# sdwyc/ROLO

Hardware: AMD Instinct MI355X
Metric: scans/sec (128k-pt frame, 20 GN iters) (higher is better)
Workload: dtype f64

## Files before the change

rolo_amd/csrc/knn_packet.hpp:

```cpp
#pragma once
#include "rolo_internal.hpp"
#include "dev_math.hpp"
#include <cfloat>
#include <climits>

#ifndef KNN_STAT
#ifdef ROLO_KNN_STATS
#define KNN_STAT(x) x
#else
#define KNN_STAT(x)
#endif
#endif

namespace rolo {
namespace {

constexpr int WALK_STACK = KNN_WALK_STACK;

ROLO_DEV float box_d2(const float4& lo, const float4& hi, const float4& q) {
  float dx = fmaxf(fmaxf(__fsub_rn(lo.x, q.x), __fsub_rn(q.x, hi.x)), 0.f);
  float dy = fmaxf(fmaxf(__fsub_rn(lo.y, q.y), __fsub_rn(q.y, hi.y)), 0.f);
  float dz = fmaxf(fmaxf(__fsub_rn(lo.z, q.z), __fsub_rn(q.z, hi.z)), 0.f);
  return __fadd_rn(__fadd_rn(__fmul_rn(dx, dx), __fmul_rn(dy, dy)), __fmul_rn(dz, dz));
}

ROLO_DEV double key_pack(float d2, int idx) {
  return __longlong_as_double((long long)(((unsigned long long)__float_as_uint(d2) << 32) | (unsigned)idx));
}
ROLO_DEV float key_d2(double k) { return __uint_as_float((unsigned)((unsigned long long)__double_as_longlong(k) >> 32)); }
ROLO_DEV int key_idx(double k) { return (int)(unsigned)((unsigned long long)__double_as_longlong(k) & 0xffffffffull); }

ROLO_DEV double vmin_f64(double a, double b) { double r; asm("v_min_f64 %0, %1, %2" : "=v"(r) : "v"(a), "v"(b)); return r; }
ROLO_DEV double vmax_f64(double a, double b) { double r; asm("v_max_f64 %0, %1, %2" : "=v"(r) : "v"(a), "v"(b)); return r; }
#ifndef ROLO_KNN_SPLIT_MINMAX
ROLO_DEV void insert_slot(double& ks, double ksm1, double c) { asm("v_min_f64 %0, %1, %0\n\tv_max_f64 %0, %2, %0" : "+&v"(ks) : "v"(c), "v"(ksm1)); }
#else
ROLO_DEV void insert_slot(double& ks, double ksm1, double c) { ks = vmax_f64(ksm1, vmin_f64(c, ks)); }
#endif
#ifndef ROLO_KNN_B1
#define ROLO_KNN_B1 15
#define ROLO_KNN_B2 10
#define ROLO_KNN_B3 5
#endif
template <int KMAX>
ROLO_DEV void insert_tiered(double (&K)[KMAX], double ck) {
  constexpr int B1 = KMAX == 20 ? ROLO_KNN_B1 : 3 * (KMAX / 4), B2 = KMAX == 20 ? ROLO_KNN_B2 : 2 * (KMAX / 4), B3 = KMAX == 20 ? ROLO_KNN_B3 : KMAX / 4;
#pragma unroll
  for (int s = KMAX - 1; s >= B1; s--) insert_slot(K[s], K[s - 1], ck);
  if (__any(ck < K[B1 - 1])) {
#pragma unroll
    for (int s = B1 - 1; s >= B2; s--) insert_slot(K[s], K[s - 1], ck);
    if (__any(ck < K[B2 - 1])) {
#pragma unroll
      for (int s = B2 - 1; s >= B3; s--) insert_slot(K[s], K[s - 1], ck);
      if (__any(ck < K[B3 - 1])) {
#pragma unroll
        for (int s = B3 - 1; s >= 1; s--) insert_slot(K[s], K[s - 1], ck);
        K[0] = vmin_f64(ck, K[0]);
      }
    }
  }
}

ROLO_DEV void sload_leaf(const float4* __restrict__ p, float4 (&pts)[KNN_LEAF]) {
#pragma unroll
  for (int u = 0; u < KNN_LEAF; u++) pts[u] = p[u];
}
ROLO_DEV void sload_node(const float4* __restrict__ p, float4& llo, float4& lhi, float4& rlo, float4& rhi) { llo = p[0]; lhi = p[1]; rlo = p[2]; rhi = p[3]; }

template <int KMAX, bool LOWER = false>
ROLO_DEV void knn_score_leaf(const float4* __restrict__ sorted, int g, const float4& q, double (&K)[KMAX], int kk, double& bkey, float& bd,
                             unsigned& n_ins, unsigned& lane_acc, unsigned& rounds, double lo = 0.0) {
  float4 pts[KNN_LEAF];
  sload_leaf(sorted + KNN_LEAF * (size_t)g, pts);
  KNN_STAT(const double bkey0 = bkey; unsigned my_acc = 0;)
#ifdef ROLO_KNN_STATS2
  unsigned my_cur = 0;
#endif
#pragma unroll
  for (int u = 0; u < KNN_LEAF; u++) {
    const float4 c = pts[u];
    const float dx = q.x - c.x, dy = q.y - c.y, dz = q.z - c.z;
    const float cd = ((dx * dx) + (dy * dy)) + (dz * dz);
    const double ck0 = key_pack(cd, __float_as_int(c.w));
    const double ck = (LOWER && !(ck0 > lo)) ? key_pack(INFINITY, INT_MAX) : ck0;
    KNN_STAT(if (__any(ck < bkey)) { n_ins++; lane_acc += (unsigned)__popcll(__ballot(ck < bkey)); })
    KNN_STAT(if (ck < bkey0) my_acc++;)
#ifdef ROLO_KNN_STATS2
    if (ck < bkey) my_cur++;
#endif
    if (ck < bkey) {
      insert_tiered<KMAX>(K, ck);
#pragma unroll
      for (int s = 0; s < KMAX; s++) if (s == kk - 1) bkey = K[s];
      bd = key_d2(bkey);
    }
  }
#ifdef ROLO_KNN_STATS
#ifdef ROLO_KNN_STATS2
  rounds += my_cur;
  (void)my_acc;
#else
  { unsigned m = my_acc;
    for (int off = 32; off > 0; off >>= 1) m = max(m, (unsigned)__shfl_xor((int)m, off, 64));
    rounds += m; }
#endif
#endif
}

template <int CTRL>
ROLO_DEV double dpp_f64(double x) {
  const long long v = __double_as_longlong(x);
  const int lo = __builtin_amdgcn_mov_dpp((int)(unsigned)(unsigned long long)v, CTRL, 0xF, 0xF, true);
  const int hi = __builtin_amdgcn_mov_dpp((int)(unsigned)((unsigned long long)v >> 32), CTRL, 0xF, 0xF, true);
  return __longlong_as_double((long long)(((unsigned long long)(unsigned)hi << 32) | (unsigned)lo));
}
template <int ST> ROLO_DEV double sub_xchg(double x) { return ST == 0 ? dpp_f64<0xB1>(x) : ST == 1 ? dpp_f64<0x4E>(x) : dpp_f64<0x141>(x); }
template <int SUB> ROLO_DEV double sub_min(double x) {
  x = vmin_f64(x, sub_xchg<0>(x));
  if (SUB >= 4) x = vmin_f64(x, sub_xchg<1>(x));
  if (SUB >= 8) x = vmin_f64(x, sub_xchg<2>(x));
  return x;
}
template <int SUB> ROLO_DEV double sub_max(double x) {
  x = vmax_f64(x, sub_xchg<0>(x));
  if (SUB >= 4) x = vmax_f64(x, sub_xchg<1>(x));
  if (SUB >= 8) x = vmax_f64(x, sub_xchg<2>(x));
  return x;
}

ROLO_DEV int xcd_contiguous_block(int b, int G, int wpb = 4) {
#ifdef ROLO_KNN_NO_XCD_REMAP
  return b;
#else
  if (G * wpb <= 2048) {
    const int x = b & 7, k = b >> 3, q = G >> 3, r = G & 7;
    return x * q + min(x, r) + k;
  }
  const int RUN = 256 / wpb, GROUP = 8 * RUN;
  if (b >= G / GROUP * GROUP) return b;
  const int grp = b / GROUP, o = b - grp * GROUP;
  return grp * GROUP + (o & 7) * RUN + (o >> 3);
#endif
}

typedef __attribute__((address_space(3))) int lds_int;

template <int KMAX, bool LOWER>
ROLO_DEV void packet_walk(const float4* __restrict__ sorted, const float4* __restrict__ boxes, int P, int g_own0, int g_own1, const float4& q, double (&K)[KMAX], int kk,
                          double& bkey, float& bd, double lo, lds_int* stk, int& sp, int h,
                          unsigned& st_nodes, unsigned& st_leaves, unsigned& st_ins, unsigned& st_lane, unsigned& st_rounds, unsigned& st_push) {
  (void)st_push;
  while (true) {
    h = __builtin_amdgcn_readfirstlane(h);
    if (h < P) {
      st_nodes++;
      float4 llo, lhi, rlo, rhi;
      sload_node(boxes + 4 * (size_t)h, llo, lhi, rlo, rhi);
      const float bl = box_d2(llo, lhi, q), br = box_d2(rlo, rhi, q);
      const bool okl = (bl <= bd) && (bl < INFINITY), okr = (br <= bd) && (br < INFINITY);
      const unsigned long long ml = __ballot(okl), mr = __ballot(okr);
      if (ml != 0ull && mr != 0ull) {
        const unsigned long long pref = __ballot((okl || okr) && (bl <= br));
        const bool left_first = 2 * __popcll(pref) >= __popcll(ml | mr);
        if (sp < WALK_STACK) { stk[sp] = left_first ? 2 * h + 1 : 2 * h; sp++; KNN_STAT(st_push++;) }
        h = left_first ? 2 * h : 2 * h + 1;
        continue;
      }
      if (ml != 0ull) { h = 2 * h; continue; }
      if (mr != 0ull) { h = 2 * h + 1; continue; }
    } else {
      const int g = h - P;
      if (g < g_own0 || g >= g_own1) {
        knn_score_leaf<KMAX, LOWER>(sorted, g, q, K, kk, bkey, bd, st_ins, st_lane, st_rounds, lo);
        st_leaves++;
      }
    }
    if (sp == 0) return;
    sp--;
    h = stk[sp];
  }
}

}
}
```

rolo_amd/csrc/knn_walk.hpp:

```cpp
#pragma once
#ifdef ROLO_KNN_STATS
#define KNN_STAT(x) x
#else
#define KNN_STAT(x)
#endif
#include "knn_packet.hpp"

namespace rolo {
namespace {

ROLO_DEV double* stage_area(const KnnCloud& cl, unsigned add) {
  double* s = cl.stage;
  if (cl.stage_epoch) {
    const unsigned long long e = __hip_atomic_load(cl.stage_epoch, __ATOMIC_RELAXED, __HIP_MEMORY_SCOPE_SYSTEM) + add;
    if (e & 1ull) s += cl.stage_alt;
  }
  return s;
}

#ifdef ROLO_KNN_STATS
__device__ unsigned g_knn_wave_rec[16384][8];
#endif

template <int KMAX>
ROLO_DEV void walk_write_lists(const KnnCloud& cl, const double (&K)[KMAX], int kk, double bkey, int qi, int j) {
  int ki[KMAX];
#pragma unroll
  for (int u = 0; u < KMAX; u++) ki[u] = key_idx(K[u]);
  const int slot0 = (KMAX == 64) ? cl.slot0 : 0;
  const int ktot = (KMAX == 64 && cl.k_total) ? cl.k_total : kk;
  if (cl.knn_idx) {
#pragma unroll
    for (int u = 0; u < KMAX; u++) if (u < kk) { cl.knn_idx[(size_t)qi * ktot + slot0 + u] = ki[u]; cl.knn_d2[(size_t)qi * ktot + slot0 + u] = key_d2(K[u]); }
  }
  if (KMAX == 64 && cl.lower) cl.lower[j] = bkey;
  int32_t* __restrict__ nbr = cl.nbr;
#pragma unroll
  for (int u = 0; u < KMAX; u++) nbr[(size_t)(slot0 + u) * cl.n_sorted + j] = ki[u];
}

template <int KMAX>
ROLO_DEV void walk_write_moments(const KnnCloud& cl, const double (&K)[KMAX], int kk, int qi, int j, int (*s_ki)[256]) {
  if (cl.knn_idx) {
#pragma unroll
    for (int u = 0; u < KMAX; u++) if (u < kk) { cl.knn_idx[(size_t)qi * kk + u] = key_idx(K[u]); cl.knn_d2[(size_t)qi * kk + u] = key_d2(K[u]); }
  }
  const int tid = threadIdx.x;
#pragma unroll
  for (int u = 0; u < KMAX; u++) s_ki[u][tid] = key_idx(K[u]);
  const float4* __restrict__ orig = cl.xyz;
  double mx = 0, my = 0, mz = 0;
#pragma unroll 5
  for (int u = 0; u < kk; u++) { const float4 p = orig[s_ki[u][tid]]; mx += (double)p.x; my += (double)p.y; mz += (double)p.z; }
  mx /= kk; my /= kk; mz /= kk;
  double cxx = 0, cxy = 0, cxz = 0, cyy = 0, cyz = 0, czz = 0;
#pragma unroll 5
  for (int u = 0; u < kk; u++) {
    const float4 p = orig[s_ki[u][tid]];
    const double ax = (double)p.x - mx, ay = (double)p.y - my, az = (double)p.z - mz;
    cxx += ax * ax; cxy += ax * ay; cxz += ax * az; cyy += ay * ay; cyz += ay * az; czz += az * az;
  }
  double* __restrict__ mom = reinterpret_cast<double*>(cl.nbr);
  const size_t pitch = (size_t)cl.n_sorted;
  mom[j] = cxx / kk; mom[pitch + j] = cxy / kk; mom[2 * pitch + j] = cxz / kk; mom[3 * pitch + j] = cyy / kk; mom[4 * pitch + j] = cyz / kk; mom[5 * pitch + j] = czz / kk;
}

#ifndef ROLO_KNN_WALK_OCC
#define ROLO_KNN_WALK_OCC 4
#endif
#ifndef ROLO_KNN_PACKET
#define ROLO_KNN_PACKET 64
#endif
#ifndef ROLO_KNN_SEED_EXTRA
#define ROLO_KNN_SEED_EXTRA 1
#endif
static_assert(ROLO_KNN_PACKET == 64, "one query per lane");

template <int KMAX, bool LOWER>
ROLO_DEV void walk_seeds(const float4* __restrict__ sorted, int g_mine0, int g_own0, int g_own1, int n_leaves, const float4& q, double (&K)[KMAX], int kk, double& bkey, float& bd, double lo,
                         unsigned& st_leaves, unsigned& st_ins, unsigned& st_lane, unsigned& st_rounds) {
  const int n_own = min(g_mine0 + 64 / KNN_LEAF, n_leaves) - g_mine0, n_before = g_mine0 - g_own0;
  for (int i = 0; i < g_own1 - g_own0; i++) {
    const int g = i < n_own ? g_mine0 + i : (i - n_own < n_before ? g_own0 + (i - n_own) : g_mine0 + (i - n_before));
    knn_score_leaf<KMAX, LOWER>(sorted, g, q, K, kk, bkey, bd, st_ins, st_lane, st_rounds, lo);
    st_leaves++;
  }
}

template <int KMAX, bool LOWER = false, bool MOMENTS = false>
__global__ __launch_bounds__(256, KMAX > 32 ? 2 : (MOMENTS ? 6 : ROLO_KNN_WALK_OCC)) void knn_walk_kernel(KnnPair A, int split, int k) {
  __shared__ int stk[4][WALK_STACK];
  __shared__ int s_ki[MOMENTS ? KMAX : 1][256];
  const int tid = threadIdx.x;
  const int wv = tid >> 6;
  const int blk = xcd_contiguous_block((int)blockIdx.x, (int)gridDim.x, 4);
  const int which = blk >= split ? 1 : 0;
  const float4* __restrict__ sorted = A.c[which].sorted;
  const float4* __restrict__ boxes = A.c[which].boxes;
  const int n_sorted = A.c[which].n_sorted, P = A.c[which].P;
  const int lane_ = tid & 63;
  const int j = A.c[which].q_begin + (blk - (which ? split : 0)) * 256 + wv * 64 + lane_;
  float4 q = make_float4(0.f, 0.f, 0.f, 0.f);
  int qi = INT_MAX;
  if (j < A.c[which].q_end) { q = sorted[j]; qi = __float_as_int(q.w); }
  const bool active = qi != INT_MAX;
  const int kk = (KMAX == 20) ? 20 : k;
  const int n_leaves = n_sorted / KNN_LEAF;
  unsigned st_nodes = 0, st_leaves = 0, st_ins = 0, st_lane = 0, st_rounds = 0, st_push = 0;

  const double sentinel = key_pack(INFINITY, INT_MAX);
  double K[KMAX];
#pragma unroll
  for (int u = 0; u < KMAX; u++) K[u] = sentinel;
  float bd = active ? INFINITY : -1.0f;
  double bkey = active ? sentinel : key_pack(0.f, 0);

  const int g_mine0 = __builtin_amdgcn_readfirstlane(j / KNN_LEAF);
  const int g_own0 = max(g_mine0 - ROLO_KNN_SEED_EXTRA, 0);
  const int g_own1 = min(g_mine0 + 64 / KNN_LEAF + ROLO_KNN_SEED_EXTRA, n_leaves);
  double lo = 0.0;
  if (LOWER && active) lo = A.c[which].lower[j];
  (void)lo;
  walk_seeds<KMAX, LOWER>(sorted, g_mine0, g_own0, g_own1, n_leaves, q, K, kk, bkey, bd, lo, st_leaves, st_ins, st_lane, st_rounds);

  int sp = 0;
  int h = 1;
#ifdef ROLO_KNN_STATS
  unsigned long long wt0;
  asm("s_memrealtime %0\n\ts_waitcnt lgkmcnt(0)\n\ts_mov_b32 %1, 1" : "=s"(wt0), "=s"(h));
#endif
  packet_walk<KMAX, LOWER>(sorted, boxes, P, g_own0, g_own1, q, K, kk, bkey, bd, lo, (lds_int*)&stk[wv][0], sp, h, st_nodes, st_leaves, st_ins, st_lane, st_rounds, st_push);
#ifdef ROLO_KNN_STATS
  { unsigned long long wt1; asm volatile("s_memrealtime %0\n\ts_waitcnt lgkmcnt(0)" : "=s"(wt1));
    unsigned st_rounds_rec = st_rounds;
#ifdef ROLO_KNN_STATS2
    for (int off = 32; off > 0; off >>= 1) st_rounds_rec = max(st_rounds_rec, (unsigned)__shfl_xor((int)st_rounds_rec, off, 64));
#endif
    const unsigned wid = blockIdx.x * 4 + (threadIdx.x >> 6);
    if ((threadIdx.x & 63) == 0 && wid < 16384) {
      g_knn_wave_rec[wid][0] = st_nodes; g_knn_wave_rec[wid][1] = st_leaves; g_knn_wave_rec[wid][2] = st_ins; g_knn_wave_rec[wid][3] = st_push;
      g_knn_wave_rec[wid][4] = (unsigned)wt0; g_knn_wave_rec[wid][5] = (unsigned)wt1; g_knn_wave_rec[wid][6] = st_lane; g_knn_wave_rec[wid][7] = st_rounds_rec;
    } }
#endif
  (void)st_nodes; (void)st_leaves; (void)st_ins; (void)st_lane; (void)st_rounds; (void)st_push;

  if (!active) return;

  if (MOMENTS) {
    walk_write_moments<KMAX>(A.c[which], K, kk, qi, j, s_ki);
    return;
  }
  walk_write_lists<KMAX>(A.c[which], K, kk, bkey, qi, j);
}

template <int ST> ROLO_DEV void merge20(double (&K)[20]) {
#pragma unroll
  for (int j = 0; j < 10; j++) {
    const double o1 = sub_xchg<ST>(K[19 - j]), o2 = sub_xchg<ST>(K[j]);
    K[j] = vmin_f64(K[j], o1);
    K[19 - j] = vmin_f64(K[19 - j], o2);
  }
#pragma unroll
  for (int d = 16; d >= 1; d >>= 1) {
#pragma unroll
    for (int p = 12; p < 32; p++) {
      if ((p & d) == 0) {
        const int x = p - 12, y = p + d - 12;
        const double lo = vmin_f64(K[x], K[y]);
        K[y] = vmax_f64(K[x], K[y]);
        K[x] = lo;
      }
    }
  }
}

template <int SUB, bool MOMENTS = false>
__global__ __launch_bounds__(256, MOMENTS ? 6 : ROLO_KNN_WALK_OCC) void knn_walk_sub_kernel(KnnPair A, int split ) {
  constexpr int SH = SUB == 2 ? 1 : 2, QPW = 64 / SUB, PPL = KNN_LEAF / SUB, KMAX = 20, E = 4 / SUB , OWN = QPW / KNN_LEAF;
  static_assert(SUB == 2 || SUB == 4, "lanes per query");
  static_assert(KNN_LEAF == 16, "a wavefront's queries are whole leaves");
  __shared__ int stk_[4][WALK_STACK];
  __shared__ int s_ki[MOMENTS ? KMAX : 1][256];
  const int tid = threadIdx.x;
  const int wv = __builtin_amdgcn_readfirstlane(tid >> 6), lane = tid & 63, sub = lane & (SUB - 1), ql = lane >> SH;
  const int blk = xcd_contiguous_block((int)blockIdx.x, (int)gridDim.x, 4);
  const int which = blk >= split ? 1 : 0;
  const KnnCloud& cl = A.c[which];
  const float4* __restrict__ sorted = cl.sorted;
  const float4* __restrict__ boxes = cl.boxes;
  const int n_sorted = cl.n_sorted, P = cl.P, n_leaves = n_sorted / KNN_LEAF;
  const int j0 = cl.q_begin + ((blk - (which ? split : 0)) * 4 + wv) * QPW;
  const int j = j0 + ql;
  float4 q = make_float4(0.f, 0.f, 0.f, 0.f);
  int qi = INT_MAX;
  if (j < cl.q_end) { q = sorted[j]; qi = __float_as_int(q.w); }
  const bool active = qi != INT_MAX;
  const double sentinel = key_pack(INFINITY, INT_MAX);
  double K[KMAX];
#pragma unroll
  for (int u = 0; u < KMAX; u++) K[u] = sentinel;
  double B = active ? sentinel : key_pack(0.f, 0);
  float bd = active ? INFINITY : -1.0f;
  auto score = [&](int g) {
    const float4* __restrict__ leaf = sorted + KNN_LEAF * (size_t)g;
    bool changed = false;
#pragma unroll
    for (int t0 = 0; t0 < PPL; t0 += 4) {
      float4 c[4];
#pragma unroll
      for (int t = 0; t < 4; t++) c[t] = leaf[(t0 + t) * SUB + sub];
#pragma unroll
      for (int t = 0; t < 4; t++) {
        const float dx = q.x - c[t].x, dy = q.y - c[t].y, dz = q.z - c[t].z;
        const float cd = ((dx * dx) + (dy * dy)) + (dz * dz);
        const double ck = key_pack(cd, __float_as_int(c[t].w));
        if (ck < B) { insert_tiered<KMAX>(K, ck); changed = true; }
      }
    }
    if (__any(changed)) {
      B = vmin_f64(vmin_f64(B, sub_min<SUB>(K[KMAX - 1])), sub_max<SUB>(K[KMAX / SUB - 1]));
      bd = key_d2(B);
    }
  };
  const int g_mine = min(j0 / KNN_LEAF, n_leaves - 1);
  const int g_own0 = max(g_mine - ROLO_KNN_SEED_EXTRA, 0), g_own1 = min(g_mine + OWN + ROLO_KNN_SEED_EXTRA, n_leaves);
  for (int g = g_mine; g < min(g_mine + OWN, n_leaves); g++) score(g);
  for (int g = g_own0; g < g_own1; g++) if (g < g_mine || g >= g_mine + OWN) score(g);
  {
    lds_int* stk = (lds_int*)&stk_[wv][0];
    int sp = 0, h = 1;
    while (true) {
      h = __builtin_amdgcn_readfirstlane(h);
      if (2 * h < P) {
        float d[E]; bool ok[E];
        float dm = INFINITY;
#pragma unroll
        for (int e = 0; e < E; e++) {
          const int c = sub * E + e;
          const float4 blo = boxes[8 * (size_t)h + 2 * c], bhi = boxes[8 * (size_t)h + 2 * c + 1];
          d[e] = box_d2(blo, bhi, q);
          ok[e] = (d[e] <= bd) && (d[e] < INFINITY);
          dm = fminf(dm, ok[e] ? d[e] : INFINITY);
        }
        dm = fminf(dm, __int_as_float(__builtin_amdgcn_mov_dpp(__float_as_int(dm), 0xB1, 0xF, 0xF, true)));
        if (SUB == 4) dm = fminf(dm, __int_as_float(__builtin_amdgcn_mov_dpp(__float_as_int(dm), 0x4E, 0xF, 0xF, true)));
        unsigned long long m[E], v[E];
#pragma unroll
        for (int e = 0; e < E; e++) { m[e] = __ballot(ok[e]); v[e] = __ballot(ok[e] && d[e] == dm); }
        int key[4];
#pragma unroll
        for (int c = 0; c < 4; c++) {
          const unsigned long long sel = (SUB == 4 ? 0x1111111111111111ull : 0x5555555555555555ull) << (c / E);
          key[c] = (m[c % E] & sel) != 0ull ? __popcll(v[c % E] & sel) * 4 + (3 - c) : -1;
        }
        auto cx = [](int& a, int& bb) { const int hi = max(a, bb), lo = min(a, bb); a = hi; bb = lo; };
        cx(key[0], key[1]); cx(key[2], key[3]); cx(key[0], key[2]); cx(key[1], key[3]); cx(key[1], key[2]);
        if (key[0] >= 0) {
#pragma unroll
          for (int r = 3; r >= 1; r--) if (key[r] >= 0 && sp < WALK_STACK) { stk[sp] = 4 * h + (3 - (key[r] & 3)); sp++; }
          h = 4 * h + (3 - (key[0] & 3));
          continue;
        }
      } else if (h < P) {
        const int c = sub & 1;
        const float4 blo = boxes[4 * (size_t)h + 2 * c], bhi = boxes[4 * (size_t)h + 2 * c + 1];
        const float d = box_d2(blo, bhi, q);
        const float o = __int_as_float(__builtin_amdgcn_mov_dpp(__float_as_int(d), 0xB1, 0xF, 0xF, true));
        const bool ok = (d <= bd) && (d < INFINITY), oko = (o <= bd) && (o < INFINITY);
        const unsigned long long m = __ballot(ok);
        const unsigned long long ml = m & 0x5555555555555555ull, mr = m & 0xaaaaaaaaaaaaaaaaull;
        if (ml != 0ull && mr != 0ull) {
          const unsigned long long pref = __ballot(c == 0 && (ok || oko) && (d <= o));
          const unsigned long long either = (ml | (mr >> 1)) & 0x5555555555555555ull;
          const bool left_first = 2 * __popcll(pref) >= __popcll(either);
          if (sp < WALK_STACK) { stk[sp] = left_first ? 2 * h + 1 : 2 * h; sp++; }
          h = left_first ? 2 * h : 2 * h + 1;
          continue;
        }
        if (ml != 0ull) { h = 2 * h; continue; }
        if (mr != 0ull) { h = 2 * h + 1; continue; }
      } else {
        const int g = h - P;
        if (g < g_own0 || g >= g_own1) score(g);
      }
      if (sp == 0) break;
      sp--;
      h = stk[sp];
    }
  }
  merge20<0>(K);
  if (SUB == 4) merge20<1>(K);
  if (MOMENTS) {
    if (active && sub == 0) walk_write_moments<KMAX>(cl, K, KMAX, qi, j, s_ki);
    return;
  }
  constexpr int NS = KMAX / SUB;
  int ki[NS];
#pragma unroll
  for (int t = 0; t < NS; t++) {
    if (SUB == 4) {
      const double k01 = sub & 1 ? K[NS + t] : K[t], k23 = sub & 1 ? K[3 * NS + t] : K[2 * NS + t];
      ki[t] = key_idx(sub & 2 ? k23 : k01);
    } else {
      ki[t] = key_idx(sub & 1 ? K[NS + t] : K[t]);
    }
  }
  if (!active) return;
  int32_t* __restrict__ nbr = cl.nbr;
#pragma unroll
  for (int t = 0; t < NS; t++) nbr[(size_t)(sub * NS + t) * n_sorted + j] = ki[t];
  if (cl.knn_idx && sub == 0) {
#pragma unroll
    for (int u = 0; u < KMAX; u++) { cl.knn_idx[(size_t)qi * KMAX + u] = key_idx(K[u]); cl.knn_d2[(size_t)qi * KMAX + u] = key_d2(K[u]); }
  }
}

#ifndef ROLO_KNN_TAIL_OCC
#define ROLO_KNN_TAIL_OCC 2
#endif
template <int KMAX, bool MOMENTS = false>
__global__ __launch_bounds__(256, ROLO_KNN_TAIL_OCC) void knn_tail_kernel(KnnPair A, int split, int k, int reg, VoxelFuse vf) {
  ROLO_TAIL_KERNEL_PRIO();
  int which, blk;
  {
    const int b = xcd_contiguous_block((int)blockIdx.x, (int)gridDim.x), nb0 = split, nb1 = (int)gridDim.x - split, m = nb0 < nb1 ? nb0 : nb1;
    if (b < 2 * m) { which = b & 1; blk = (b >> 1) + (which ? split : 0); }
    else { which = nb0 > nb1 ? 0 : 1; blk = m + (b - 2 * m) + (which ? split : 0); }
  }
  const KnnCloud& cl = A.c[which];
  const int n_sorted = cl.n_sorted;
  const int j = cl.q_begin + (blk - (which ? split : 0)) * 256 + threadIdx.x;
  const bool fuse = vf.enabled && which == vf.which && !cl.stage;
  float4 sp = make_float4(0.f, 0.f, 0.f, 0.f);
  int qi = INT_MAX;
  if (j < cl.q_end) { sp = cl.sorted[j]; qi = __float_as_int(sp.w); }
  const bool act = qi != INT_MAX;
  if (!act && !fuse) return;
  int vox_id = -1;
  if (fuse && act) { const int slot = vf.tgt_slot[qi]; if (slot >= 0) vox_id = slot_id(vf.tab, (unsigned)slot); }
  double c6[6] = {0, 0, 0, 0, 0, 0};
  if (act && MOMENTS) {
    const size_t pitch = (size_t)n_sorted;
    const double* __restrict__ cv = reinterpret_cast<const double*>(cl.nbr);
    const double m0 = cv[j], m1 = cv[pitch + j], m2 = cv[2 * pitch + j], m3 = cv[3 * pitch + j], m4 = cv[4 * pitch + j], m5 = cv[5 * pitch + j];
    if (cl.stage) {
      double* o = stage_area(cl, 1) + (size_t)(j / cl.chunk) * cl.seg + cl.stage_off + (size_t)(j % cl.chunk) * 6;
      knn_covariance_finish(m0, m1, m2, m3, m4, m5, 1, 0, reg, o, c6);
    } else {
      knn_covariance_finish(m0, m1, m2, m3, m4, m5, cl.n, qi, reg, cl.cov, c6, cl.nrm);
    }
  } else if (act) {
    const int32_t* __restrict__ nbr = cl.nbr;
    int ki[KMAX];
#pragma unroll
    for (int u = 0; u < KMAX; u++) ki[u] = nbr[(size_t)u * n_sorted + j];
    if (cl.stage) {
      double* o = stage_area(cl, 1) + (size_t)(j / cl.chunk) * cl.seg + cl.stage_off + (size_t)(j % cl.chunk) * 6;
      knn_covariance_tail<KMAX>(ki, (KMAX == 20) ? 20 : k, cl.xyz, 1, 0, reg, o, c6);
    } else {
      knn_covariance_tail<KMAX>(ki, (KMAX == 20) ? 20 : k, cl.xyz, cl.n, qi, reg, cl.cov, c6, cl.nrm);
    }
  }
#ifdef ROLO_VOXEL_ACCUM_WAVE
  if (fuse) accumulate_point(vf.tab, vox_id, sp, c6, fix_scales(cl.n, vf.counters), true, const_cast<int*>(vf.counters) + 1);
#else
  if (fuse) accumulate_point_wg<256>(vf.tab, vox_id, sp, c6, fix_scales(cl.n, vf.counters), const_cast<int*>(vf.counters) + 1);
#endif
}

__global__ __launch_bounds__(256) void knn_tail_loop_kernel(KnnPair A, int split, int k, int reg, VoxelFuse vf) {
  const int blk = xcd_contiguous_block((int)blockIdx.x, (int)gridDim.x);
  const int which = blk >= split ? 1 : 0;
  const KnnCloud& cl = A.c[which];
  const int j = cl.q_begin + (blk - (which ? split : 0)) * 256 + threadIdx.x;
  const bool fuse = vf.enabled && which == vf.which && !cl.stage;
  float4 sp = make_float4(0.f, 0.f, 0.f, 0.f);
  int qi = INT_MAX;
  if (j < cl.q_end) { sp = cl.sorted[j]; qi = __float_as_int(sp.w); }
  const bool act = qi != INT_MAX;
  if (!act && !fuse) return;
  double c6[6] = {0, 0, 0, 0, 0, 0};
  if (act) {
    if (cl.stage) {
      double* o = stage_area(cl, 1) + (size_t)(j / cl.chunk) * cl.seg + cl.stage_off + (size_t)(j % cl.chunk) * 6;
      knn_covariance_tail_loop(cl.nbr, (size_t)cl.n_sorted, j, k, cl.xyz, 1, 0, reg, o, c6);
    } else {
      knn_covariance_tail_loop(cl.nbr, (size_t)cl.n_sorted, j, k, cl.xyz, cl.n, qi, reg, cl.cov, c6, cl.nrm);
    }
  }
  if (fuse) {
    int id = -1;
    if (act) { const int slot = vf.tgt_slot[qi]; if (slot >= 0) id = slot_id(vf.tab, (unsigned)slot); }
    accumulate_point_wg<256>(vf.tab, id, sp, c6, fix_scales(cl.n, vf.counters), const_cast<int*>(vf.counters) + 1);
  }
}

__global__ __launch_bounds__(256) void knn_unstage_kernel(KnnPair A, int split, int own_only, VoxelFuse vf) {
  const int which = (int)blockIdx.x >= split ? 1 : 0;
  const KnnCloud& cl = A.c[which];
  const int j = (own_only ? cl.q_begin : 0) + ((int)blockIdx.x - (which ? split : 0)) * 256 + threadIdx.x;
  const bool fuse = vf.enabled && which == vf.which;
  float4 sp = make_float4(0.f, 0.f, 0.f, 0.f);
  int qi = INT_MAX;
  if (j < (own_only ? cl.q_end : cl.n_sorted)) { sp = cl.sorted[j]; qi = __float_as_int(sp.w); }
  const bool act = qi != INT_MAX;
  if (!act && !fuse) return;
  double c6[6] = {0, 0, 0, 0, 0, 0};
  if (act) {
    const double* __restrict__ o = stage_area(cl, 0) + (size_t)(j / cl.chunk) * cl.seg + cl.stage_off + (size_t)(j % cl.chunk) * 6;
    const size_t pitch = (size_t)cl.n;
#pragma unroll
    for (int v = 0; v < 6; v++) { c6[v] = o[v]; cl.cov[v * pitch + qi] = c6[v]; }
  }
  if (fuse) {
    int id = -1;
    if (act) { const int slot = vf.tgt_slot[qi]; if (slot >= 0) id = slot_id(vf.tab, (unsigned)slot); }
    accumulate_point_wg<256>(vf.tab, id, sp, c6, fix_scales(cl.n, vf.counters), const_cast<int*>(vf.counters) + 1);
  }
}

}
}
```

Baseline: 4237.

## Seed KNN lists with branch-free sorting-network merges instead of per-point inserts

Seed-leaf scoring now sorts each chunk of 8 (or 4) candidate keys with a fixed sorting network and merges it into the top-20 list with bitonic clean passes, replacing per-point tiered insertion with its data-dependent branches and ballots. The bound is refreshed once after all seed leaves instead of after every insert. The aim is to cut wavefront divergence and per-point branch overhead during seeding. In exchange it always does the full compare-exchange work even when a candidate would be rejected, and it skips the early bound tightening that could prune later points.

```diff
diff --git a/rolo_amd/csrc/knn_packet.hpp b/rolo_amd/csrc/knn_packet.hpp
--- a/rolo_amd/csrc/knn_packet.hpp
+++ b/rolo_amd/csrc/knn_packet.hpp
@@ -1,6 +1,7 @@
 #pragma once
 #include "rolo_internal.hpp"
 #include "dev_math.hpp"
+#include "knn_seed_net.hpp"
 #include <cfloat>
 #include <climits>
 
@@ -106,6 +107,31 @@
     rounds += m; }
 #endif
 #endif
+}
+
+struct KeyMin { ROLO_DEV double operator()(double a, double b) const { return vmin_f64(a, b); } };
+struct KeyMax { ROLO_DEV double operator()(double a, double b) const { return vmax_f64(a, b); } };
+
+template <int NB, int STRIDE, class P>
+ROLO_DEV void seed_chunk(const P& p, int first, const float4& q, double (&K)[20]) {
+  double b[NB];
+#pragma unroll
+  for (int u = 0; u < NB; u++) {
+    const float4 c = p[first + u * STRIDE];
+    const float dx = q.x - c.x, dy = q.y - c.y, dz = q.z - c.z;
+    const float cd = ((dx * dx) + (dy * dy)) + (dz * dz);
+    b[u] = key_pack(cd, __float_as_int(c.w));
+  }
+  if constexpr (NB == 8) seednet::sort8(b, KeyMin(), KeyMax()); else seednet::sort4(b, KeyMin(), KeyMax());
+  seednet::merge_chunk<NB>(K, b, KeyMin(), KeyMax());
+}
+
+ROLO_DEV void knn_seed_leaf(const float4* __restrict__ sorted, int g, const float4& q, double (&K)[20]) {
+  static_assert(KNN_LEAF == 16, "two chunks of 8");
+  float4 pts[KNN_LEAF];
+  sload_leaf(sorted + KNN_LEAF * (size_t)g, pts);
+  seed_chunk<8, 1>(pts, 0, q, K);
+  seed_chunk<8, 1>(pts, 8, q, K);
 }
 
 template <int CTRL>
diff --git a/rolo_amd/csrc/knn_seed_net.hpp b/rolo_amd/csrc/knn_seed_net.hpp
--- /dev/null
+++ b/rolo_amd/csrc/knn_seed_net.hpp
@@ -0,0 +1,61 @@
+#pragma once
+
+#if defined(__HIPCC__) || defined(__CUDACC__)
+#define ROLO_NET_FN __host__ __device__ __forceinline__
+#define ROLO_NET_UNROLL _Pragma("unroll")
+#else
+#define ROLO_NET_FN inline
+#define ROLO_NET_UNROLL
+#endif
+
+namespace rolo {
+namespace seednet {
+
+template <class T, class Min, class Max>
+ROLO_NET_FN void cx(T& a, T& b, Min mn, Max mx) {
+  const T lo = mn(a, b);
+  b = mx(a, b);
+  a = lo;
+}
+
+template <class T, class Min, class Max>
+ROLO_NET_FN void sort8(T (&b)[8], Min mn, Max mx) {
+  constexpr int net[19][2] = {{0, 2}, {1, 3}, {4, 6}, {5, 7}, {0, 4}, {1, 5}, {2, 6}, {3, 7}, {0, 1}, {2, 3}, {4, 5}, {6, 7}, {2, 4}, {3, 5}, {1, 4}, {3, 6}, {1, 2}, {3, 4}, {5, 6}};
+ROLO_NET_UNROLL
+  for (int c = 0; c < 19; c++) cx(b[net[c][0]], b[net[c][1]], mn, mx);
+}
+
+template <class T, class Min, class Max>
+ROLO_NET_FN void sort4(T (&b)[4], Min mn, Max mx) {
+  cx(b[0], b[1], mn, mx); cx(b[2], b[3], mn, mx); cx(b[0], b[2], mn, mx); cx(b[1], b[3], mn, mx); cx(b[1], b[2], mn, mx);
+}
+
+template <int N, int OFF, bool DESC, class T, int KN, class Min, class Max>
+ROLO_NET_FN void bitonic_clean(T (&K)[KN], Min mn, Max mx) {
+  constexpr int P2 = N <= 4 ? 4 : N <= 8 ? 8 : N <= 16 ? 16 : 32, PAD = P2 - N;
+  static_assert(N <= 32 && OFF + N <= KN, "run inside the list");
+ROLO_NET_UNROLL
+  for (int d = P2 / 2; d >= 1; d >>= 1) {
+ROLO_NET_UNROLL
+    for (int p = PAD; p < P2; p++) {
+      if ((p & d) == 0) {
+        if (DESC) cx(K[OFF + p + d - PAD], K[OFF + p - PAD], mn, mx);
+        else cx(K[OFF + p - PAD], K[OFF + p + d - PAD], mn, mx);
+      }
+    }
+  }
+}
+
+template <int NB, class T, class Min, class Max>
+ROLO_NET_FN void merge_chunk(T (&K)[20], const T (&b)[NB], Min mn, Max mx) {
+  static_assert(NB == 8 || NB == 4, "chunk size");
+ROLO_NET_UNROLL
+  for (int i = 0; i < NB; i++) K[20 - NB + i] = mn(K[20 - NB + i], b[NB - 1 - i]);
+  bitonic_clean<NB, 20 - NB, true>(K, mn, mx);
+  bitonic_clean<20, 0, false>(K, mn, mx);
+}
+template <class T, class Min, class Max>
+ROLO_NET_FN void merge8(T (&K)[20], const T (&b)[8], Min mn, Max mx) { merge_chunk<8>(K, b, mn, mx); }
+
+}
+}
diff --git a/rolo_amd/csrc/knn_walk.hpp b/rolo_amd/csrc/knn_walk.hpp
--- a/rolo_amd/csrc/knn_walk.hpp
+++ b/rolo_amd/csrc/knn_walk.hpp
@@ -77,13 +77,17 @@
 static_assert(ROLO_KNN_PACKET == 64, "one query per lane");
 
 template <int KMAX, bool LOWER>
-ROLO_DEV void walk_seeds(const float4* __restrict__ sorted, int g_mine0, int g_own0, int g_own1, int n_leaves, const float4& q, double (&K)[KMAX], int kk, double& bkey, float& bd, double lo,
+ROLO_DEV void walk_seeds(const float4* __restrict__ sorted, int g_mine0, int g_own0, int g_own1, int n_leaves, const float4& q, bool active, double (&K)[KMAX], int kk, double& bkey, float& bd, double lo,
                          unsigned& st_leaves, unsigned& st_ins, unsigned& st_lane, unsigned& st_rounds) {
   const int n_own = min(g_mine0 + 64 / KNN_LEAF, n_leaves) - g_mine0, n_before = g_mine0 - g_own0;
   for (int i = 0; i < g_own1 - g_own0; i++) {
     const int g = i < n_own ? g_mine0 + i : (i - n_own < n_before ? g_own0 + (i - n_own) : g_mine0 + (i - n_before));
-    knn_score_leaf<KMAX, LOWER>(sorted, g, q, K, kk, bkey, bd, st_ins, st_lane, st_rounds, lo);
+    if constexpr (KMAX == 20 && !LOWER) knn_seed_leaf(sorted, g, q, K);
+    else knn_score_leaf<KMAX, LOWER>(sorted, g, q, K, kk, bkey, bd, st_ins, st_lane, st_rounds, lo);
     st_leaves++;
+  }
+  if constexpr (KMAX == 20 && !LOWER) {
+    if (active) { bkey = K[KMAX - 1]; bd = key_d2(bkey); }
   }
 }
 
@@ -121,7 +125,7 @@
   double lo = 0.0;
   if (LOWER && active) lo = A.c[which].lower[j];
   (void)lo;
-  walk_seeds<KMAX, LOWER>(sorted, g_mine0, g_own0, g_own1, n_leaves, q, K, kk, bkey, bd, lo, st_leaves, st_ins, st_lane, st_rounds);
+  walk_seeds<KMAX, LOWER>(sorted, g_mine0, g_own0, g_own1, n_leaves, q, active, K, kk, bkey, bd, lo, st_leaves, st_ins, st_lane, st_rounds);
 
   int sp = 0;
   int h = 1;
@@ -160,18 +164,7 @@
     K[j] = vmin_f64(K[j], o1);
     K[19 - j] = vmin_f64(K[19 - j], o2);
   }
-#pragma unroll
-  for (int d = 16; d >= 1; d >>= 1) {
-#pragma unroll
-    for (int p = 12; p < 32; p++) {
-      if ((p & d) == 0) {
-        const int x = p - 12, y = p + d - 12;
-        const double lo = vmin_f64(K[x], K[y]);
-        K[y] = vmax_f64(K[x], K[y]);
-        K[x] = lo;
-      }
-    }
-  }
+  seednet::bitonic_clean<20, 0, false>(K, KeyMin(), KeyMax());
 }
 
 template <int SUB, bool MOMENTS = false>
@@ -224,8 +217,9 @@
   };
   const int g_mine = min(j0 / KNN_LEAF, n_leaves - 1);
   const int g_own0 = max(g_mine - ROLO_KNN_SEED_EXTRA, 0), g_own1 = min(g_mine + OWN + ROLO_KNN_SEED_EXTRA, n_leaves);
-  for (int g = g_mine; g < min(g_mine + OWN, n_leaves); g++) score(g);
-  for (int g = g_own0; g < g_own1; g++) if (g < g_mine || g >= g_mine + OWN) score(g);
+  for (int g = g_own0; g < g_own1; g++) seed_chunk<PPL, SUB>(sorted + KNN_LEAF * (size_t)g, sub, q, K);
+  B = vmin_f64(vmin_f64(B, sub_min<SUB>(K[KMAX - 1])), sub_max<SUB>(K[KMAX / SUB - 1]));
+  if (active) bd = key_d2(B);
   {
     lds_int* stk = (lds_int*)&stk_[wv][0];
     int sp = 0, h = 1;
```

Result: faster. 4429 (median of 6 runs) (+4.5%).
